# xinntao/EDVR

Measured on AMD Instinct MI355X. Metric: EDVR-L x4 5-frame 720p clips/sec, higher is better.
Workload: dtype fp32 emulated as 2xf16 (hi+lo, 22-bit operands, 4 cross products), fp32 accumulate; 1 GPU; EDVR-L x4, 5 frames, 180x320 LR -> 720x1280, batch 10/GPU, inference; clips_per_gpu=10, global_clips=10, parallelism=clip-sharded x1, no data-path collective, world_size=1, backend=single process

## Files before the change

edvr_amd/_lib.py:

```python
import ctypes
import os

_HERE = os.path.dirname(os.path.abspath(__file__))
LIB_PATH = os.environ.get('EDVR_AMD_LIB') or os.path.join(_HERE, 'lib', 'libedvr_amd.so')

c_float_p = ctypes.c_void_p
i32, i64, f32, sz = ctypes.c_int, ctypes.c_int64, ctypes.c_float, ctypes.c_size_t
vp = ctypes.c_void_p


class ConvDesc(ctypes.Structure):
    _fields_ = [
        ('x1', vp), ('x2', vp), ('c1', i32), ('c2', i32), ('x1_img_stride', i64), ('x2_img_stride', i64),
        ('x2_div', i32), ('x2_mul', i32), ('x2_add', i32), ('n', i32), ('h', i32), ('w', i32), ('wpk', vp),
        ('bias', vp), ('co', i32), ('ks', i32), ('stride', i32), ('act', i32), ('act_from', i32), ('res1', vp),
        ('res2', vp), ('res1_img_stride', i64), ('res2_img_stride', i64), ('y', vp), ('y_img_stride', i64),
        ('out_mode', i32), ('algo', i32), ('gate', vp), ('gate_img_stride', i64), ('gate_slope', f32), ('y_scale', f32),
        ('wpk_f4', vp), ('abs_sum', vp), ('abs_sum_channels', i32), ('wpk_f4s', vp), ('x_amax', vp), ('y_amax', vp),
        ('pre', vp), ('pre_img_stride', i64), ('pre_div', i32), ('pre_mul', i32), ('pre_add', i32), ('pre_n', i32), ('wpk_ds', vp),
    ]


PROTOTYPES = {
    'edvr_version': (ctypes.c_char_p, []),
    'edvr_last_error': (ctypes.c_char_p, []),
    'edvr_check_device': (i32, []),
    'edvr_conv2d_packed_weight_elems': (sz, [i32, i32, i32]),
    'edvr_conv2d_pack_weight_f32': (i32, [vp, vp, i32, i32, i32, i32, vp]),
    'edvr_conv2d_packed_weight_f4_elems': (sz, [i32, i32]),
    'edvr_conv2d_pack_weight_f4_f32': (i32, [vp, vp, i32, i32, i32, vp]),
    'edvr_conv2d_packed_weight_f4s_elems': (sz, [i32, i32]),
    'edvr_conv2d_pack_weight_f4s_f32': (i32, [vp, vp, i32, i32, i32, vp]),
    'edvr_conv2d_packed_weight_1x1s_elems': (sz, [i32, i32]),
    'edvr_conv2d_pack_weight_1x1s_f32': (i32, [vp, vp, i32, i32, vp]),
    'edvr_conv2d_packed_weight_ds_elems': (sz, [i32, i32, i32]),
    'edvr_conv2d_pack_weight_ds_f32': (i32, [vp, vp, i32, i32, i32, vp]),
    'edvr_amax_f32': (i32, [vp, vp, i32, i64, i64, vp]),
    'edvr_pack_job_bytes': (sz, []),
    'edvr_conv2d_pack_weights_multi': (i32, [vp, i32, i32, i32, vp]),
    'edvr_conv2d_f32': (i32, [ctypes.POINTER(ConvDesc), vp]),
    'edvr_conv2d_kernel': (i32, [ctypes.POINTER(ConvDesc)]),
    'edvr_conv2d_gate_supported': (i32, [ctypes.POINTER(ConvDesc)]),
    'edvr_conv2d_abs_sum_supported': (i32, [ctypes.POINTER(ConvDesc)]),
    'edvr_conv2d_y_amax_supported': (i32, [ctypes.POINTER(ConvDesc)]),
    'edvr_conv2d_pre_supported': (i32, [ctypes.POINTER(ConvDesc)]),
    'edvr_conv2d_f4s_set_lean': (i32, [i32]),
    'edvr_conv2d_f4s_lean_items': (i32, [ctypes.POINTER(ConvDesc)]),
    'edvr_conv2d_kernel_name': (i32, [ctypes.POINTER(ConvDesc), ctypes.c_char_p, sz]),
    'edvr_conv2d_executed_flops': (i32, [ctypes.POINTER(ConvDesc), ctypes.POINTER(ctypes.c_double)]),
    'edvr_dcnv2_fwd_ws_bytes': (sz, [i32] * 12),
    'edvr_dcnv2_fwd_f32': (i32, [vp] * 6 + [i32] * 12 + [i64, i64, i32, i32, vp, sz, vp]),
    'edvr_dcnv2_fwd_split_f32': (i32, [vp] * 6 + [i32] * 12 + [i64, i64, i32, i32, vp, sz, vp, vp]),
    'edvr_dcnv2_fwd_split_applies': (i32, [vp] + [i32] * 13),
    'edvr_dcnv2_fwd_kernel_name': (i32, [vp] + [i32] * 13 + [ctypes.c_char_p, sz]),
    'edvr_dcnv2_bwd_ws_bytes': (sz, [i32] * 12),
    'edvr_dcnv2_any_ws_bytes': (sz, [i32] * 13),
    'edvr_dcnv2_fwd_any': (i32, [i32] + [vp] * 6 + [i32] * 12 + [i64, i64, vp, sz, vp]),
    'edvr_dcnv2_bwd_any': (i32, [i32] + [vp] * 10 + [i32] * 12 + [i64, i64, i64, i64, vp, sz, vp]),
    'edvr_psnr_sse_f32': (i32, [vp, vp, vp, i32, i32, i32, i32, i64, i64, i32, i32, i32, vp]),
    'edvr_ssim_partials': (sz, [i32, i32, i32]),
    'edvr_ssim_f32': (i32, [vp, vp, vp, i32, i32, i32, i32, i64, i64, i32, i32, vp]),
    'edvr_niqe_blocks': (sz, [i32, i32, i32]),
    'edvr_niqe_moments_f32': (i32, [vp, vp, i32, i32, i32, i32, i64, i32, vp]),
    'edvr_niqe_moments_u8': (i32, [vp, vp, i32, i32, i32, i64, i32, vp]),
    'edvr_frames_u8_to_f32': (i32, [vp, vp, i32, i32, i32, i32, vp, i32, vp]),
    'edvr_gather_images_f32': (i32, [vp, vp, vp, vp, i32, vp, i32, i32, vp]),
    'edvr_upsample4x_add_u8': (i32, [vp, vp, vp, i32, i32, i32, vp]),
# ... 108 lines not shown
```

edvr_amd/csrc/conv1x1_s.hip:

```cpp
#include <cstdlib>

#include "common.h"
#include "pack.h"

namespace edvr {

typedef float f32x16 __attribute__((ext_vector_type(16)));
typedef int c1s_i32x4 __attribute__((ext_vector_type(4)));
typedef _Float16 c1s_f16x8 __attribute__((ext_vector_type(8)));

struct Conv1x1SArgs {
  edvr_conv2d_desc d;
  const unsigned *wq;
  int ci, cop, co_start;
  int seg_shift;
};

template <int MT>
__global__ __launch_bounds__(256, 2) void conv1x1_split_kernel(const Conv1x1SArgs a) {
  constexpr int CK = 64, MB = 32 * MT, DEPTH = 8, NW = CK * MB / 4 / 256;
  constexpr int RSRC_FLAGS = 0x00020000;
  constexpr int OOB = (int)0x80000000;
  __shared__ __attribute__((aligned(16))) unsigned wsm[2][CK * MB];
  const edvr_conv2d_desc &d = a.d;
  const float s_x = split_scale(__builtin_bit_cast(float, __builtin_amdgcn_readfirstlane(__builtin_bit_cast(int, *d.x_amax))));
  const float inv_sw = __builtin_bit_cast(float, __builtin_amdgcn_readfirstlane((int)a.wq[1]));
  const int tid = threadIdx.x, lane = tid & 63, half = lane >> 5, j = lane & 31;
  const int wave = __builtin_amdgcn_readfirstlane(tid >> 6);
  const int hw = d.h * d.w;
  const int img = blockIdx.z, co_blk = a.co_start + blockIdx.y * MB;
  const int p = (blockIdx.x * 4 + wave) * 32 + j;
  const bool p_ok = p < hw;

  auto uniform_ptr = [&](const float *ptr) {
    const uint64_t pv = reinterpret_cast<uint64_t>(ptr);
    return ((uint64_t)(uint32_t)__builtin_amdgcn_readfirstlane((int)(pv >> 32)) << 32) | (uint32_t)__builtin_amdgcn_readfirstlane((int)(uint32_t)pv);
  };
  const uint64_t b1 = uniform_ptr(d.x1 + (int64_t)img * d.x1_img_stride);
  uint64_t b2 = b1;
  if (d.x2) {
    const int i2 = d.x2_div > 0 ? (img / d.x2_div) * d.x2_mul + d.x2_add : img;
    b2 = uniform_ptr(d.x2 + (int64_t)i2 * d.x2_img_stride);
  }
  const int voff = p_ok ? (4 * half * hw + p) * 4 : OOB;
  const int real_steps = (d.c1 + d.c2) / 8;
  const int seg_mask = (1 << a.seg_shift) - 1;
  const int64_t plane_bytes = (int64_t)hw * 4;
  auto load_b = [&](int s, float (&v)[4]) {
    const int c = 8 * s;
    const bool first = c < d.c1;
    const int cc = first ? c : c - d.c1;
    const uint64_t base = (first ? b1 : b2) + (uint64_t)((int64_t)(cc & ~seg_mask) * plane_bytes);
    const __amdgpu_buffer_rsrc_t rs = __builtin_amdgcn_make_buffer_rsrc(reinterpret_cast<void *>(base), (short)0, 0x7fffffff, RSRC_FLAGS);
    const bool ok = s < real_steps;
#pragma unroll
    for (int i = 0; i < 4; ++i)
      v[i] = __builtin_bit_cast(float, __builtin_amdgcn_raw_buffer_load_b32(rs, ok ? voff : OOB, ok ? ((cc & seg_mask) + i) * hw * 4 : 0, 0));
  };

  const int quads_total = (d.c1 + d.c2 + 3) / 4;
  c1s_i32x4 wr[NW];
  auto w_load = [&](int c0) {
#pragma unroll
    for (int i = 0; i < NW; ++i) {
      const int e = tid + i * 256, q = e / MB, col = e - q * MB;
      const bool ok = c0 / 4 + q < quads_total;
      const c1s_i32x4 v = *reinterpret_cast<const c1s_i32x4 *>(a.wq + 16 + ((int64_t)(ok ? c0 / 4 + q : 0) * a.cop + co_blk + col) * 4);
      wr[i] = ok ? v : c1s_i32x4{0, 0, 0, 0};
    }
  };
  auto w_commit = [&](int buf) {
#pragma unroll
    for (int i = 0; i < NW; ++i) *reinterpret_cast<c1s_i32x4 *>(&wsm[buf][(tid + i * 256) * 4]) = wr[i];
  };

  f32x16 acc[MT];
#pragma unroll
  for (int m = 0; m < MT; ++m)
#pragma unroll
    for (int r = 0; r < 16; ++r) acc[m][r] = 0.f;
  float bq[DEPTH][4];
#pragma unroll
  for (int k = 0; k < DEPTH; ++k) load_b(k, bq[k]);
  w_load(0);
  w_commit(0);
  __syncthreads();

  const int chunks = a.ci / CK;
  for (int ch = 0; ch < chunks; ++ch) {
    const int buf = ch & 1;
    const bool more = ch + 1 < chunks;
    if (more) w_load((ch + 1) * CK);
    const unsigned *ws = wsm[buf] + (half * MB + j) * 4;
#pragma unroll
    for (int s = 0; s < CK / 8; ++s) {
      c1s_i32x4 av[MT];
#pragma unroll
      for (int m = 0; m < MT; ++m) av[m] = *reinterpret_cast<const c1s_i32x4 *>(ws + ((2 * s) * MB + m * 32) * 4);
      unsigned pk[4];
      split4_f16x2(bq[s % DEPTH], s_x, pk);
      load_b(ch * (CK / 8) + s + DEPTH, bq[s % DEPTH]);
      c1s_i32x4 b, br;
#pragma unroll
      for (int q = 0; q < 4; ++q) {
        b[q] = (int)pk[q];
        br[q] = (int)__builtin_amdgcn_alignbit(pk[q], pk[q], 16);
      }
#pragma unroll
      for (int m = 0; m < MT; ++m) acc[m] = __builtin_amdgcn_mfma_f32_32x32x16_f16(__builtin_bit_cast(c1s_f16x8, av[m]), __builtin_bit_cast(c1s_f16x8, b), acc[m], 0, 0, 0);
#pragma unroll
      for (int m = 0; m < MT; ++m) acc[m] = __builtin_amdgcn_mfma_f32_32x32x16_f16(__builtin_bit_cast(c1s_f16x8, av[m]), __builtin_bit_cast(c1s_f16x8, br), acc[m], 0, 0, 0);
      if (s == CK / 16 && more) w_commit(buf ^ 1);
    }
    asm volatile("s_waitcnt lgkmcnt(0)\n\ts_barrier" ::: "memory");
  }

  const float unscale = inv_sw / s_x;
  const float slope = d.act == EDVR_ACT_LRELU ? 0.1f : (d.act == EDVR_ACT_RELU ? 0.f : 1.f);
  const bool sig = d.act == EDVR_ACT_SIGMOID;
  float *y = d.y + (int64_t)img * d.y_img_stride;
  const float *q1 = d.res1 ? d.res1 + (int64_t)img * d.res1_img_stride : nullptr;
  const float *q2 = d.res2 ? d.res2 + (int64_t)img * d.res2_img_stride : nullptr;
  unsigned vmax = 0u;
  if (p_ok) {
#pragma unroll
    for (int m = 0; m < MT; ++m)
#pragma unroll
      for (int r = 0; r < 16; ++r) {
        const int co = co_blk + m * 32 + (r & 3) + 8 * (r >> 2) + 4 * half;
        if (co < d.co) {
          float v = __builtin_fmaf(acc[m][r], unscale, d.bias ? d.bias[co] : 0.f);
          if (co >= d.act_from) v = sig ? __builtin_amdgcn_rcpf(1.f + __expf(-v)) : fmaxf(v, slope * v);
          const int64_t off = (int64_t)co * hw + p;
          if (q1) v += q1[off];
          if (q2) v += q2[off];
          y[off] = v;
          vmax = max(vmax, __builtin_bit_cast(unsigned, v) & 0x7fffffffu);
        }
      }
  }
  if (d.y_amax) {
#pragma unroll
    for (int sh = 32; sh > 0; sh >>= 1) vmax = max(vmax, (unsigned)__shfl_xor((int)vmax, sh));
    if (lane == 0) publish_amax(d.y_amax, vmax);
  }
}

static bool conv1x1_split_enabled() {
  static const bool on = []() {
    const char *e = getenv("EDVR_CONV1X1_SPLIT");
    return !(e && e[0] == '0');
  }();
  return on;
}

bool conv1x1_split_eligible(const edvr_conv2d_desc &d) {
  if (!conv1x1_split_enabled() || !d.wpk_f4s || !d.x_amax || d.algo == EDVR_CONV_DIRECT) return false;
  if (!conv1x1_eligible(d)) return false;
  if ((d.c1 & 7) || (d.c2 & 7)) return false;
  return (int64_t)d.h * d.w * 32 < ((int64_t)1 << 31);
}

int conv1x1_split_launch(const edvr_conv2d_desc &d, hipStream_t stream) {
  EDVR_REQUIRE((reinterpret_cast<uintptr_t>(d.wpk_f4s) & 15) == 0, "conv1x1_split: packed weights must be 16-byte aligned");
  Conv1x1SArgs a;
  a.d = d;
  a.wq = reinterpret_cast<const unsigned *>(d.wpk_f4s);
  a.ci = ((d.c1 + d.c2 + 63) / 64) * 64;
  a.cop = (d.co + 127) / 128 * 128;
  const int hw = d.h * d.w;
  a.seg_shift = 30;
  while (((int64_t)1 << a.seg_shift) * hw * 4 >= ((int64_t)1 << 31)) --a.seg_shift;
  if (a.seg_shift < 3) a.seg_shift = 3;
  const int full = d.co / 128, rem_tiles = cdiv(d.co - full * 128, 32);
  if (full > 0) {
    a.co_start = 0;
    hipLaunchKernelGGL((conv1x1_split_kernel<4>), dim3(cdiv(hw, 128), full, d.n), dim3(256), 0, stream, a);
  }
  if (rem_tiles > 0) {
    a.co_start = full * 128;
    const dim3 grid(cdiv(hw, 128), 1, d.n);
    if (rem_tiles == 1) hipLaunchKernelGGL((conv1x1_split_kernel<1>), grid, dim3(256), 0, stream, a);
    else if (rem_tiles == 2) hipLaunchKernelGGL((conv1x1_split_kernel<2>), grid, dim3(256), 0, stream, a);
    else hipLaunchKernelGGL((conv1x1_split_kernel<3>), grid, dim3(256), 0, stream, a);
  }
  return check_launch("conv1x1_split_kernel");
}

}

extern "C" {

size_t edvr_conv2d_packed_weight_1x1s_elems(int co, int ci) {
  if (co <= 0 || ci <= 0) return 0;
  return 16 + (size_t)((ci + 63) / 64 * 16) * ((co + 127) / 128 * 128) * 4;
}

int edvr_conv2d_pack_weight_1x1s_f32(const float *w, void *wpk, int co, int ci, edvr_stream_t stream_) {
  using namespace edvr;
  EDVR_REQUIRE(w && wpk && co > 0 && ci > 0, "pack_weight_1x1s: bad arguments");
  EDVR_REQUIRE((reinterpret_cast<uintptr_t>(wpk) & 15) == 0, "pack_weight_1x1s: wpk must be 16-byte aligned");
  hipStream_t stream = as_stream(stream_);
  unsigned *wq = static_cast<unsigned *>(wpk);
  const int cop = (co + 127) / 128 * 128, quads = (ci + 63) / 64 * 16;
  return conv_split_pack(w, wq, co, ci, 1, cop, quads, stream);
}

}
```

edvr_amd/edvr_arch.py:

```python
import torch
from torch import nn

from . import functional as F_
from .arch_util import DCNv2Pack, ResidualBlockNoBN, make_layer, warn_offset_absmean

LRELU = F_.ACT_LRELU


def _conv3(cin, cout, stride=1):
    return nn.Conv2d(cin, cout, 3, stride, 1)


class PCDAlignment(nn.Module):

    def __init__(self, num_feat=64, deformable_groups=8):
        super().__init__()
        self.offset_conv1, self.offset_conv2, self.offset_conv3 = nn.ModuleDict(), nn.ModuleDict(), nn.ModuleDict()
        self.dcn_pack, self.feat_conv = nn.ModuleDict(), nn.ModuleDict()
        for lv in (3, 2, 1):
            key = f'l{lv}'
            self.offset_conv1[key] = _conv3(2 * num_feat, num_feat)
            if lv == 3:
                self.offset_conv2[key] = _conv3(num_feat, num_feat)
            else:
# ... 43 lines not shown
        self.temporal_attn1 = _conv3(num_feat, num_feat)
        self.temporal_attn2 = _conv3(num_feat, num_feat)
        self.feat_fusion = nn.Conv2d(num_frame * num_feat, num_feat, 1, 1)
        self.max_pool = nn.MaxPool2d(3, stride=2, padding=1)
        self.avg_pool = nn.AvgPool2d(3, stride=2, padding=1)
        self.spatial_attn1 = nn.Conv2d(num_frame * num_feat, num_feat, 1)
        self.spatial_attn2 = nn.Conv2d(num_feat * 2, num_feat, 1)
        self.spatial_attn3 = _conv3(num_feat, num_feat)
        self.spatial_attn4 = nn.Conv2d(num_feat, num_feat, 1)
        self.spatial_attn5 = _conv3(num_feat, num_feat)
        self.spatial_attn_l1 = nn.Conv2d(num_feat, num_feat, 1)
        self.spatial_attn_l2 = _conv3(num_feat * 2, num_feat)
        self.spatial_attn_l3 = _conv3(num_feat, num_feat)
        self.spatial_attn_add1 = nn.Conv2d(num_feat, num_feat, 1)
        self.spatial_attn_add2 = nn.Conv2d(num_feat, num_feat, 1)
        self.lrelu = nn.LeakyReLU(negative_slope=0.1, inplace=True)
        self.upsample = nn.Upsample(scale_factor=2, mode='bilinear', align_corners=False)

    def forward(self, aligned_feat):
        return self.spatial(self.temporal(aligned_feat))

    def temporal(self, aligned_feat, pair=False):
        b, t, c, h, w = aligned_feat.shape
        alias = F_.ops.carry_bound
        emb_ref = F_.conv(self.temporal_attn1, alias(aligned_feat[:, self.center_frame_idx], aligned_feat))
        emb = F_.conv(self.temporal_attn2, alias(aligned_feat.reshape(b * t, c, h, w), aligned_feat)).view(b, t, -1, h, w)
        if pair:
            mod, mod_rev = F_.tsa_temporal_pair(emb, emb_ref, aligned_feat)
            return alias(mod.view(b, t * c, h, w), mod), alias(mod_rev.view(b, t * c, h, w), mod_rev)
        mod = F_.tsa_temporal(emb, emb_ref, aligned_feat)
        return alias(mod.view(b, t * c, h, w), mod)

    def spatial(self, mod):
        feat = F_.conv(self.feat_fusion, mod, act=LRELU)
        attn = F_.conv(self.spatial_attn1, mod, act=LRELU)
        attn = F_.conv(self.spatial_attn2, F_.pool_maxavg(attn), act=LRELU)
        lvl = F_.conv(self.spatial_attn_l1, attn, act=LRELU)
        lvl = F_.conv(self.spatial_attn_l2, F_.pool_maxavg(lvl), act=LRELU)
        lvl = F_.upsample2x(F_.conv(self.spatial_attn_l3, lvl, act=LRELU))
        attn = F_.conv(self.spatial_attn3, attn, act=LRELU, res1=lvl)
        attn = F_.upsample2x(F_.conv(self.spatial_attn4, attn, act=LRELU))
        attn = F_.conv(self.spatial_attn5, attn)
        attn_add = F_.conv(self.spatial_attn_add2, F_.conv(self.spatial_attn_add1, attn, act=LRELU))
        return F_.tsa_combine(feat, attn, attn_add)


class PredeblurModule(nn.Module):

    def __init__(self, num_in_ch=3, num_feat=64, hr_in=False):
        super().__init__()
        self.hr_in = hr_in
        self.conv_first = _conv3(num_in_ch, num_feat)
        if hr_in:
            self.stride_conv_hr1 = _conv3(num_feat, num_feat, 2)
            self.stride_conv_hr2 = _conv3(num_feat, num_feat, 2)
        self.stride_conv_l2 = _conv3(num_feat, num_feat, 2)
        self.stride_conv_l3 = _conv3(num_feat, num_feat, 2)
        self.resblock_l3 = ResidualBlockNoBN(num_feat=num_feat)
        self.resblock_l2_1 = ResidualBlockNoBN(num_feat=num_feat)
        self.resblock_l2_2 = ResidualBlockNoBN(num_feat=num_feat)
        self.resblock_l1 = nn.ModuleList([ResidualBlockNoBN(num_feat=num_feat) for _ in range(5)])
        self.upsample = nn.Upsample(scale_factor=2, mode='bilinear', align_corners=False)
        self.lrelu = nn.LeakyReLU(negative_slope=0.1, inplace=True)

    def forward(self, x):
        f1 = F_.conv(self.conv_first, x, act=LRELU)
        if self.hr_in:
            f1 = F_.conv(self.stride_conv_hr2, F_.conv(self.stride_conv_hr1, f1, act=LRELU), act=LRELU)
# ... 250 lines not shown
```

edvr_amd/functional.py:

```python
import math
import os

import torch

from . import ops
from .ops import ACT_LRELU, ACT_NONE, ACT_RELU, ACT_SIGMOID, OUT_NCHW, OUT_PIXEL_SHUFFLE2


def _conv_geometry(m):
    ks, st = m.kernel_size, m.stride
    if (ks[0] != ks[1] or ks[0] not in (1, 3) or st[0] != st[1] or st[0] not in (1, 2) or (ks[0] == 1 and st[0] != 1)
            or tuple(m.padding) != (ks[0] // 2, ks[0] // 2) or tuple(m.dilation) != (1, 1) or m.groups != 1):
        raise NotImplementedError(
            f'edvr_amd conv kernel supports 3x3 (stride 1/2, pad 1) and 1x1 convolutions, dilation 1, groups 1; got {m}')
    return ks[0], st[0]


def _needs_grad(*ts):
    return torch.is_grad_enabled() and any(t is not None and t.requires_grad for t in ts)


def conv(m, x, *, x2=None, x2_map=None, act=ACT_NONE, act_from=0, res1=None, res2=None, out_mode=OUT_NCHW, y_scale=1.0,
         abs_sum_channels=0, ci_range=None, use_bias=True, pre=None, pre_map=None, out=None):
    ks, stride = _conv_geometry(m)
# ... 1 lines not shown
        raise ValueError(f'expected a 4-D input, got {tuple(x.shape)}')
    cin = x.shape[1] + (x2.shape[1] if x2 is not None else 0)
    want = m.in_channels if ci_range is None else ci_range[1] - ci_range[0]
    if cin != want:
        raise RuntimeError(f'expected {want} input channels, got {cin}')
    ops.require_gpu(x, x2, m.weight)
    if _needs_grad(x, x2, m.weight, m.bias, res1, res2, pre):
        from . import autograd as ag
        assert abs_sum_channels == 0
        if ci_range is not None or not use_bias or pre is not None or out is not None:
            raise NotImplementedError('ci_range / use_bias / pre / out are inference-only arguments of conv()')
        return ag.conv(m, x, x2, x2_map, act, act_from, res1, res2, out_mode, ks, stride, y_scale)
    wpk = ops.pack_conv_weight(m.weight, ci_range=ci_range)
    f4 = ops.F4_INFERENCE and ks == 3 and stride == 1 and cin >= 32 and m.out_channels >= 48
    f4s = f4 and ops.F4S_INFERENCE and x.shape[3] % 4 == 0
    wf4 = ops.pack_conv_weight(m.weight, f4=True, ci_range=ci_range) if (f4 and not f4s) else None
    wf4s = ops.pack_conv_weight(m.weight, f4s=True, ci_range=ci_range) if f4s else None
    if ops.F4S_INFERENCE and ks == 1 and stride == 1 and cin >= 320 and x.shape[1] % 8 == 0 and cin % 8 == 0:
        wf4s = ops.pack_conv_weight(m.weight, f4s=True, ci_range=ci_range)
    wds = None
    if ops.F4S_INFERENCE and m.out_channels > 4 and (x2 is None or x.shape[1] % 4 == 0) and (
            (ks == 3 and (stride == 2 or cin <= 8)) or (ks == 1 and cin < 320)):
        wds = ops.pack_conv_weight(m.weight, ds=True, ci_range=ci_range)
    bias = m.bias.detach() if (m.bias is not None and use_bias) else None
    r = ops.conv2d(x, wpk, bias, m.out_channels, ks, x2=x2, x2_map=x2_map, stride=stride, act=act, act_from=act_from,
                   res1=res1, res2=res2, out_mode=out_mode, y_scale=y_scale, wpk_f4=wf4, abs_sum_channels=abs_sum_channels,
                   wpk_f4s=wf4s, pre=pre, pre_map=pre_map, out=out, wpk_ds=wds)
    y = r[0] if abs_sum_channels > 0 else r
    if ops.F4S_INFERENCE and ops.get_bound(y) is None:
        ops.linear_bound(y, m.weight, m.bias, (x, x2), (res1, res2, pre), scale=y_scale, floor=1.0 if act == ACT_SIGMOID else 0.0)
    return r


PRE_SPLIT = os.environ.get('EDVR_CONV_PRE', '1') != '0'
PRE_SPLIT_MIN_ITEMS = None


def _conv_items(n, h, w, co):
    return n * -(-co // 64) * min(-(-w // 64) * -(-h // 8), -(-w // 32) * -(-h // 16))


def conv_shared_x2(m, x, x2, x2_map, act=ACT_NONE):
    if PRE_SPLIT and x2_map is not None and x2_map[0] > 1 and not _needs_grad(x, x2, m.weight, m.bias):
        ks, stride = _conv_geometry(m)
        (n, c1, h, w), c2, co = x.shape, x2.shape[1], m.out_channels
        f4 = ops.F4_INFERENCE and ks == 3 and stride == 1 and min(c1, c2) >= 32 and co >= 48
        min_items = PRE_SPLIT_MIN_ITEMS if PRE_SPLIT_MIN_ITEMS is not None else torch.cuda.get_device_properties(x.device).multi_processor_count
        if f4 and _conv_items(n, h, w, co) > min_items and ops.conv_pre_supported(n, c1, h, w, co, ops.F4S_INFERENCE and w % 4 == 0):
            div, mul, add = x2_map
            shared = (n - 1) // div + 1
            sel = x2[add:add + 1] if (mul == 0 or shared == 1) else x2[add:add + (shared - 1) * mul + 1:mul]
            p = conv(m, ops.carry_bound(sel, x2), ci_range=(c1, c1 + c2), use_bias=False)
            return conv(m, x, act=act, ci_range=(0, c1), pre=p, pre_map=(div, 0 if sel.shape[0] == 1 else 1, 0))
    return conv(m, x, x2=x2, x2_map=x2_map, act=act)


def offset_mask_conv_stats(conv_offset, feat):
    co = conv_offset.out_channels
    if _needs_grad(feat, conv_offset.weight, conv_offset.bias):
        om = offset_mask_conv(conv_offset, feat)
        return om, ops.abs_stats_per_image(om.detach()[:, :2 * co // 3])
    return conv(conv_offset, feat, act=ACT_SIGMOID, act_from=2 * co // 3, abs_sum_channels=2 * co // 3)


def offset_mask_conv(conv_offset, feat):
    co = conv_offset.out_channels
# ... 113 lines not shown
```

edvr_amd/ops.py:

```python
import ctypes
import os
import weakref

import torch

from . import _lib
from ._lib import (ACT_LRELU, ACT_NONE, ACT_RELU, ACT_SIGMOID, CONV_AUTO, CONV_DIRECT, CONV_WINOGRAD, CONV_WINOGRAD_F4, CONV_WINOGRAD_F4S, OUT_NCHW,
                   OUT_PIXEL_SHUFFLE2)


def _stream():
    return ctypes.c_void_p(torch.cuda.current_stream().cuda_stream)


def _ptr(t):
    return ctypes.c_void_p(t.data_ptr()) if t is not None else ctypes.c_void_p(0)


def require_gpu(*tensors, dtypes=(torch.float32,)):
    seen = None
    for t in tensors:
        if t is None:
            continue
        if not t.is_cuda:
# ... 542 lines not shown
        else:
            d.wpk_f4s, d.wpk_ds, d.x_amax = None, None, None
    sums = None
    if abs_sum_channels > 0 and L.edvr_conv2d_abs_sum_supported(ctypes.byref(d)):
        sums = torch.zeros(2, n, dtype=torch.float32, device=x1.device)
        d.abs_sum, d.abs_sum_channels = _ptr(sums), int(abs_sum_channels)
    name, flops, nbytes, executed = 'conv2d', 0.0, 0.0, None
    if LAUNCH_HOOK is not None:
        buf = ctypes.create_string_buffer(96)
        L.edvr_conv2d_kernel_name(ctypes.byref(d), buf, 96)
        name = buf.value.decode()
        ex = ctypes.c_double(0.0)
        if L.edvr_conv2d_executed_flops(ctypes.byref(d), ctypes.byref(ex)) == 0:
            executed = ex.value
        flops = 2.0 * n * ho * wo * co * (c1 + d.c2) * ks * ks
        nbytes = 4.0 * (n * (c1 + d.c2) * h * w + n * co * ho * wo * (1 + (res1 is not None) + (res2 is not None) + (gate is not None) + (pre is not None))
                        + co * (c1 + d.c2) * ks * ks)
    _run(name, lambda: _lib.check(L.edvr_conv2d_f32(ctypes.byref(d), _stream()), 'edvr_conv2d_f32'), flops, nbytes, executed)
    if y_bound is not None:
        set_bound(out, y_bound)
    else:
        void_bound(out)
    if abs_sum_channels > 0:
        if sums is None:
            return out, abs_stats_per_image(out[:, :abs_sum_channels])
        step = max(1, n // 4)
        sel = out[::step, :abs_sum_channels]
        r = abs_stats_per_image(sel)
        sums[1, ::step] = r[1] * (float(n) / sel.shape[0])
        return out, sums
    return out


def conv_pre_supported(n, c, h, w, co, f4s, algo=None):
    d = _lib.ConvDesc()
    d.c1, d.n, d.h, d.w, d.co, d.ks, d.stride = c, n, h, w, co, 3, 1
    d.algo = CONV_ALGO if algo is None else algo
    any_ptr = ctypes.addressof(d) & ~15
    if f4s:
        d.wpk_f4s = d.x_amax = any_ptr
    else:
        d.wpk_f4 = any_ptr
    return bool(_lib.lib().edvr_conv2d_pre_supported(ctypes.byref(d)))


def conv_gate_supported(n, c, h, w, co, algo=None):
    d = _lib.ConvDesc()
    d.c1, d.n, d.h, d.w, d.co, d.ks, d.stride = c, n, h, w, co, 3, 1
    d.algo = CONV_ALGO if algo is None else algo
    return bool(_lib.lib().edvr_conv2d_gate_supported(ctypes.byref(d)))


def _ones_mask(offset):
    return torch.ones(offset.shape[0], offset.shape[1] // 2, offset.shape[2], offset.shape[3], dtype=offset.dtype, device=offset.device)


def dcnv1_forward(x, offset, weight, stride, pad, dil, groups, dg, halo_hint=0, out=None):
    if require_gpu(x, offset, weight, dtypes=tuple(DCN_DTYPES)) != torch.float32:
        return dcnv2_forward(x, offset, _ones_mask(offset), weight, None, stride, pad, dil, groups, dg, out=out)
    L = _lib.lib()
    offset = _as_planes(offset)
    dims = _dcn_dims(x, weight, stride, pad, dil, groups, dg)
    B, C, H, W, Co, kh, kw = dims[:7]
    ho, wo = offset.shape[2], offset.shape[3]
    if out is not None:
        if tuple(out.shape) != (B, Co, ho, wo) or out.dtype != torch.float32 or not out.is_contiguous() or out.device != x.device:
# ... 1228 lines not shown
```

include/edvr_amd.h:

```cpp
#ifndef EDVR_AMD_H
#define EDVR_AMD_H

#include <stddef.h>
#include <stdint.h>

#ifdef __cplusplus
extern "C" {
#endif

#define EDVR_OK 0
#define EDVR_ERR_ARG (-1)
#define EDVR_ERR_UNSUPPORTED (-2)
#define EDVR_ERR_LAUNCH (-3)
#define EDVR_ERR_WORKSPACE (-4)

typedef void *edvr_stream_t;

const char *edvr_version(void);
const char *edvr_last_error(void);
int edvr_check_device(void);

#define EDVR_ACT_NONE 0
#define EDVR_ACT_RELU 1
#define EDVR_ACT_LRELU 2
// ... 30 lines not shown
  const float *res1;
  const float *res2;
  int64_t res1_img_stride, res2_img_stride;
  float *y;
  int64_t y_img_stride;
  int out_mode;
  int algo;
  const float *gate;
  int64_t gate_img_stride;
  float gate_slope;
  float y_scale;
  const float *wpk_f4;
  float *abs_sum;
  int abs_sum_channels;
  const void *wpk_f4s;
  const float *x_amax;
  float *y_amax;
  const float *pre;
  int64_t pre_img_stride;
  int pre_div, pre_mul, pre_add;
  int pre_n;
  const void *wpk_ds;
} edvr_conv2d_desc;

size_t edvr_conv2d_packed_weight_elems(int co, int ci, int ks);
int edvr_conv2d_pack_weight_f32(const float *w, float *wpk, int co, int ci, int ks, int transpose_flip,
                                edvr_stream_t stream);
size_t edvr_conv2d_packed_weight_f4_elems(int co, int ci);
int edvr_conv2d_pack_weight_f4_f32(const float *w, float *wpk_f4, int co, int ci, int transpose_flip, edvr_stream_t stream);
size_t edvr_conv2d_packed_weight_f4s_elems(int co, int ci);
int edvr_conv2d_pack_weight_f4s_f32(const float *w, void *wpk_f4s, int co, int ci, int transpose_flip, edvr_stream_t stream);
size_t edvr_conv2d_packed_weight_1x1s_elems(int co, int ci);
int edvr_conv2d_pack_weight_1x1s_f32(const float *w, void *wpk_1x1s, int co, int ci, edvr_stream_t stream);
size_t edvr_conv2d_packed_weight_ds_elems(int co, int ci, int ks);
int edvr_conv2d_pack_weight_ds_f32(const float *w, void *wpk_ds, int co, int ci, int ks, edvr_stream_t stream);
int edvr_amax_f32(const float *x, float *amax, int n, int64_t per_img, int64_t img_stride, edvr_stream_t stream);
size_t edvr_pack_job_bytes(void);
int edvr_conv2d_pack_weights_multi(const void *jobs, int n_jobs, int total_blocks, int split_parity, edvr_stream_t stream);
int edvr_conv2d_f32(const edvr_conv2d_desc *d, edvr_stream_t stream);
#define EDVR_CONV_KERNEL_SMALL 0
#define EDVR_CONV_KERNEL_F4S 1
#define EDVR_CONV_KERNEL_F4 2
#define EDVR_CONV_KERNEL_F2 3
#define EDVR_CONV_KERNEL_1X1_SPLIT 4
#define EDVR_CONV_KERNEL_1X1_STREAM 5
#define EDVR_CONV_KERNEL_DIRECT_SPLIT 6
#define EDVR_CONV_KERNEL_DIRECT 7
int edvr_conv2d_kernel(const edvr_conv2d_desc *d);
int edvr_conv2d_gate_supported(const edvr_conv2d_desc *d);
int edvr_conv2d_y_amax_supported(const edvr_conv2d_desc *d);
int edvr_conv2d_abs_sum_supported(const edvr_conv2d_desc *d);
int edvr_conv2d_pre_supported(const edvr_conv2d_desc *d);
int edvr_conv2d_f4s_set_lean(int on);
int edvr_conv2d_f4s_lean_items(const edvr_conv2d_desc *d);
int edvr_conv2d_kernel_name(const edvr_conv2d_desc *d, char *buf, size_t buf_len);
int edvr_conv2d_executed_flops(const edvr_conv2d_desc *d, double *flops);

#define EDVR_HW(h, w) ((int)(h) | (((int)(w) + 1) << 16))

size_t edvr_dcnv2_fwd_ws_bytes(int B, int C, int H, int W, int Co, int kh, int kw, int stride, int pad, int dil,
                               int groups, int dg);
int edvr_dcnv2_fwd_f32(const float *x, const float *offset, const float *mask, const float *weight,
                       const float *bias, float *y, int B, int C, int H, int W, int Co, int kh, int kw, int stride,
                       int pad, int dil, int groups, int dg, int64_t offset_bstride, int64_t mask_bstride, int act,
                       int halo_hint, void *ws, size_t ws_bytes, edvr_stream_t stream);

// ... 214 lines not shown
```

Measured before the change: 106.8 clips/s.

## Fuse TSA feat_fusion and spatial_attn1 1x1 convs into one two-head kernel

Adds a two-head variant of the split-f16 1x1 conv kernel that reads the shared input once and computes both the feat_fusion and spatial_attn1 outputs in one launch, each with its own weights, bias, activation and amax slot. The TSA fusion module now calls conv_pair instead of two separate convs. The goal is to halve input reads and drop a launch for these two large 1x1 convs over the concatenated frame features. In exchange, the workgroup now holds up to eight 32-channel tiles, so chunk size drops to 32 and register pressure rises, which may reduce occupancy.

Result: no change. 107.2 clips/s (median of 6 runs) (+0.4%).

```diff
diff --git a/edvr_amd/_lib.py b/edvr_amd/_lib.py
--- a/edvr_amd/_lib.py
+++ b/edvr_amd/_lib.py
@@ -33,6 +33,8 @@
     'edvr_conv2d_pack_weight_f4s_f32': (i32, [vp, vp, i32, i32, i32, vp]),
     'edvr_conv2d_packed_weight_1x1s_elems': (sz, [i32, i32]),
     'edvr_conv2d_pack_weight_1x1s_f32': (i32, [vp, vp, i32, i32, vp]),
+    'edvr_conv1x1_split_heads_supported': (i32, [ctypes.POINTER(ConvDesc), ctypes.POINTER(ConvDesc)]),
+    'edvr_conv1x1_split_heads_f32': (i32, [ctypes.POINTER(ConvDesc), ctypes.POINTER(ConvDesc), vp]),
     'edvr_conv2d_packed_weight_ds_elems': (sz, [i32, i32, i32]),
     'edvr_conv2d_pack_weight_ds_f32': (i32, [vp, vp, i32, i32, i32, vp]),
     'edvr_amax_f32': (i32, [vp, vp, i32, i64, i64, vp]),
diff --git a/edvr_amd/csrc/conv1x1_s.hip b/edvr_amd/csrc/conv1x1_s.hip
--- a/edvr_amd/csrc/conv1x1_s.hip
+++ b/edvr_amd/csrc/conv1x1_s.hip
@@ -14,11 +14,18 @@
   const unsigned *wq;
   int ci, cop, co_start;
   int seg_shift;
+  const unsigned *wq2;
+  const float *bias2;
+  float *y2, *y2_amax;
+  int64_t y2_img_stride;
+  int co2, cop2, act2, act_from2, mt1;
 };
 
-template <int MT>
+template <int MT, int HEADS>
 __global__ __launch_bounds__(256, 2) void conv1x1_split_kernel(const Conv1x1SArgs a) {
-  constexpr int CK = 64, MB = 32 * MT, DEPTH = 8, NW = CK * MB / 4 / 256;
+  constexpr int CK = MT > 4 ? 32 : 64, MB = 32 * MT, DEPTH = 8, NW = CK * MB / 4 / 256;
+  constexpr int SPC = CK / 8, CPI = DEPTH / SPC;
+  static_assert(HEADS == 2 || MT <= 4, "one head: up to four tiles per workgroup, further blocks on grid.y");
   constexpr int RSRC_FLAGS = 0x00020000;
   constexpr int OOB = (int)0x80000000;
   __shared__ __attribute__((aligned(16))) unsigned wsm[2][CK * MB];
@@ -65,7 +72,13 @@
     for (int i = 0; i < NW; ++i) {
       const int e = tid + i * 256, q = e / MB, col = e - q * MB;
       const bool ok = c0 / 4 + q < quads_total;
-      const c1s_i32x4 v = *reinterpret_cast<const c1s_i32x4 *>(a.wq + 16 + ((int64_t)(ok ? c0 / 4 + q : 0) * a.cop + co_blk + col) * 4);
+      c1s_i32x4 v;
+      if constexpr (HEADS == 2) {
+        const bool h2 = col >= 32 * a.mt1;
+        v = *reinterpret_cast<const c1s_i32x4 *>((h2 ? a.wq2 : a.wq) + 16 + ((int64_t)(ok ? c0 / 4 + q : 0) * (h2 ? a.cop2 : a.cop) + (h2 ? col - 32 * a.mt1 : col)) * 4);
+      } else {
+        v = *reinterpret_cast<const c1s_i32x4 *>(a.wq + 16 + ((int64_t)(ok ? c0 / 4 + q : 0) * a.cop + co_blk + col) * 4);
+      }
       wr[i] = ok ? v : c1s_i32x4{0, 0, 0, 0};
     }
   };
@@ -87,34 +100,93 @@
   __syncthreads();
 
   const int chunks = a.ci / CK;
-  for (int ch = 0; ch < chunks; ++ch) {
-    const int buf = ch & 1;
-    const bool more = ch + 1 < chunks;
-    if (more) w_load((ch + 1) * CK);
-    const unsigned *ws = wsm[buf] + (half * MB + j) * 4;
-#pragma unroll
-    for (int s = 0; s < CK / 8; ++s) {
-      c1s_i32x4 av[MT];
-#pragma unroll
-      for (int m = 0; m < MT; ++m) av[m] = *reinterpret_cast<const c1s_i32x4 *>(ws + ((2 * s) * MB + m * 32) * 4);
-      unsigned pk[4];
-      split4_f16x2(bq[s % DEPTH], s_x, pk);
-      load_b(ch * (CK / 8) + s + DEPTH, bq[s % DEPTH]);
-      c1s_i32x4 b, br;
-#pragma unroll
-      for (int q = 0; q < 4; ++q) {
-        b[q] = (int)pk[q];
-        br[q] = (int)__builtin_amdgcn_alignbit(pk[q], pk[q], 16);
-      }
-#pragma unroll
-      for (int m = 0; m < MT; ++m) acc[m] = __builtin_amdgcn_mfma_f32_32x32x16_f16(__builtin_bit_cast(c1s_f16x8, av[m]), __builtin_bit_cast(c1s_f16x8, b), acc[m], 0, 0, 0);
-#pragma unroll
-      for (int m = 0; m < MT; ++m) acc[m] = __builtin_amdgcn_mfma_f32_32x32x16_f16(__builtin_bit_cast(c1s_f16x8, av[m]), __builtin_bit_cast(c1s_f16x8, br), acc[m], 0, 0, 0);
-      if (s == CK / 16 && more) w_commit(buf ^ 1);
+  for (int it = 0; it < a.ci / (8 * DEPTH); ++it) {
+#pragma unroll
+    for (int c = 0; c < CPI; ++c) {
+      const int ch = it * CPI + c;
+      const int buf = ch & 1;
+      const bool more = ch + 1 < chunks;
+      if (more) w_load((ch + 1) * CK);
+      const unsigned *ws = wsm[buf] + (half * MB + j) * 4;
+#pragma unroll
+      for (int s = 0; s < SPC; ++s) {
+        constexpr int MG = MT > 4 ? 4 : MT;
+        c1s_i32x4 av[MT];
+#pragma unroll
+        for (int m = 0; m < MG; ++m) av[m] = *reinterpret_cast<const c1s_i32x4 *>(ws + ((2 * s) * MB + m * 32) * 4);
+        unsigned pk[4];
+        split4_f16x2(bq[c * SPC + s], s_x, pk);
+        load_b(ch * SPC + s + DEPTH, bq[c * SPC + s]);
+        c1s_i32x4 b, br;
+#pragma unroll
+        for (int q = 0; q < 4; ++q) {
+          b[q] = (int)pk[q];
+          br[q] = (int)__builtin_amdgcn_alignbit(pk[q], pk[q], 16);
+        }
+        constexpr bool LATE = MT == 7;
+        if constexpr (!LATE) {
+#pragma unroll
+          for (int m = MG; m < MT; ++m) av[m] = *reinterpret_cast<const c1s_i32x4 *>(ws + ((2 * s) * MB + m * 32) * 4);
+        }
+#pragma unroll
+        for (int m0 = 0; m0 < MT; m0 += MG) {
+          if constexpr (LATE) {
+            if (m0 > 0) {
+#pragma unroll
+              for (int m = MG; m < MT; ++m) av[m] = *reinterpret_cast<const c1s_i32x4 *>(ws + ((2 * s) * MB + m * 32) * 4);
+            }
+          }
+#pragma unroll
+          for (int m = m0; m < m0 + MG && m < MT; ++m) acc[m] = __builtin_amdgcn_mfma_f32_32x32x16_f16(__builtin_bit_cast(c1s_f16x8, av[m]), __builtin_bit_cast(c1s_f16x8, b), acc[m], 0, 0, 0);
+#pragma unroll
+          for (int m = m0; m < m0 + MG && m < MT; ++m) acc[m] = __builtin_amdgcn_mfma_f32_32x32x16_f16(__builtin_bit_cast(c1s_f16x8, av[m]), __builtin_bit_cast(c1s_f16x8, br), acc[m], 0, 0, 0);
+        }
+        if (s == SPC / 2 && more) w_commit(buf ^ 1);
+      }
+      asm volatile("s_waitcnt lgkmcnt(0)\n\ts_barrier" ::: "memory");
     }
-    asm volatile("s_waitcnt lgkmcnt(0)\n\ts_barrier" ::: "memory");
-  }
-
+  }
+
+  if constexpr (HEADS == 2) {
+    const float inv_sw2 = __builtin_bit_cast(float, __builtin_amdgcn_readfirstlane((int)a.wq2[1]));
+    unsigned vmax[2] = {0u, 0u};
+    if (p_ok) {
+#pragma unroll
+      for (int m = 0; m < MT; ++m) {
+        const bool h2 = m >= a.mt1;
+        const float unscale = (h2 ? inv_sw2 : inv_sw) / s_x;
+        const int act = h2 ? a.act2 : d.act, act_from = h2 ? a.act_from2 : d.act_from, co_n = h2 ? a.co2 : d.co;
+        const float slope = act == EDVR_ACT_LRELU ? 0.1f : (act == EDVR_ACT_RELU ? 0.f : 1.f);
+        const bool sig = act == EDVR_ACT_SIGMOID;
+        const float *bias = h2 ? a.bias2 : d.bias;
+        float *y = h2 ? a.y2 + (int64_t)img * a.y2_img_stride : d.y + (int64_t)img * d.y_img_stride;
+        unsigned vm = 0u;
+#pragma unroll
+        for (int r = 0; r < 16; ++r) {
+          const int co = (h2 ? m - a.mt1 : m) * 32 + (r & 3) + 8 * (r >> 2) + 4 * half;
+          if (co < co_n) {
+            float v = __builtin_fmaf(acc[m][r], unscale, bias ? bias[co] : 0.f);
+            if (co >= act_from) v = sig ? __builtin_amdgcn_rcpf(1.f + __expf(-v)) : fmaxf(v, slope * v);
+            y[(int64_t)co * hw + p] = v;
+            vm = max(vm, __builtin_bit_cast(unsigned, v) & 0x7fffffffu);
+          }
+        }
+        vmax[0] = max(vmax[0], h2 ? 0u : vm);
+        vmax[1] = max(vmax[1], h2 ? vm : 0u);
+      }
+    }
+#pragma unroll
+    for (int hd = 0; hd < 2; ++hd) {
+      float *slot = hd ? a.y2_amax : d.y_amax;
+      if (slot) {
+        unsigned v = vmax[hd];
+#pragma unroll
+        for (int sh = 32; sh > 0; sh >>= 1) v = max(v, (unsigned)__shfl_xor((int)v, sh));
+        if (lane == 0) publish_amax(slot, v);
+      }
+    }
+    return;
+  }
   const float unscale = inv_sw / s_x;
   const float slope = d.act == EDVR_ACT_LRELU ? 0.1f : (d.act == EDVR_ACT_RELU ? 0.f : 1.f);
   const bool sig = d.act == EDVR_ACT_SIGMOID;
@@ -161,9 +233,8 @@
   return (int64_t)d.h * d.w * 32 < ((int64_t)1 << 31);
 }
 
-int conv1x1_split_launch(const edvr_conv2d_desc &d, hipStream_t stream) {
-  EDVR_REQUIRE((reinterpret_cast<uintptr_t>(d.wpk_f4s) & 15) == 0, "conv1x1_split: packed weights must be 16-byte aligned");
-  Conv1x1SArgs a;
+static Conv1x1SArgs conv1x1_split_args(const edvr_conv2d_desc &d) {
+  Conv1x1SArgs a = {};
   a.d = d;
   a.wq = reinterpret_cast<const unsigned *>(d.wpk_f4s);
   a.ci = ((d.c1 + d.c2 + 63) / 64) * 64;
@@ -172,19 +243,72 @@
   a.seg_shift = 30;
   while (((int64_t)1 << a.seg_shift) * hw * 4 >= ((int64_t)1 << 31)) --a.seg_shift;
   if (a.seg_shift < 3) a.seg_shift = 3;
+  return a;
+}
+
+int conv1x1_split_launch(const edvr_conv2d_desc &d, hipStream_t stream) {
+  EDVR_REQUIRE((reinterpret_cast<uintptr_t>(d.wpk_f4s) & 15) == 0, "conv1x1_split: packed weights must be 16-byte aligned");
+  Conv1x1SArgs a = conv1x1_split_args(d);
+  const int hw = d.h * d.w;
   const int full = d.co / 128, rem_tiles = cdiv(d.co - full * 128, 32);
   if (full > 0) {
     a.co_start = 0;
-    hipLaunchKernelGGL((conv1x1_split_kernel<4>), dim3(cdiv(hw, 128), full, d.n), dim3(256), 0, stream, a);
+    hipLaunchKernelGGL((conv1x1_split_kernel<4, 1>), dim3(cdiv(hw, 128), full, d.n), dim3(256), 0, stream, a);
   }
   if (rem_tiles > 0) {
     a.co_start = full * 128;
     const dim3 grid(cdiv(hw, 128), 1, d.n);
-    if (rem_tiles == 1) hipLaunchKernelGGL((conv1x1_split_kernel<1>), grid, dim3(256), 0, stream, a);
-    else if (rem_tiles == 2) hipLaunchKernelGGL((conv1x1_split_kernel<2>), grid, dim3(256), 0, stream, a);
-    else hipLaunchKernelGGL((conv1x1_split_kernel<3>), grid, dim3(256), 0, stream, a);
+    if (rem_tiles == 1) hipLaunchKernelGGL((conv1x1_split_kernel<1, 1>), grid, dim3(256), 0, stream, a);
+    else if (rem_tiles == 2) hipLaunchKernelGGL((conv1x1_split_kernel<2, 1>), grid, dim3(256), 0, stream, a);
+    else hipLaunchKernelGGL((conv1x1_split_kernel<3, 1>), grid, dim3(256), 0, stream, a);
   }
   return check_launch("conv1x1_split_kernel");
+}
+
+static bool conv1x1_split_takes(const edvr_conv2d_desc &d) {
+  if (!conv1x1_split_enabled() || !d.x1 || !d.y || !d.wpk_f4s || !d.x_amax || (reinterpret_cast<uintptr_t>(d.wpk_f4s) & 15)) return false;
+  if (d.ks != 1 || d.stride != 1 || d.out_mode != EDVR_OUT_NCHW || d.gate || d.pre || d.abs_sum) return false;
+  if (d.y_scale != 0.f && d.y_scale != 1.f) return false;
+  if (d.n <= 0 || d.n > 65535 || d.h <= 0 || d.w <= 0 || d.co <= 0 || d.c1 <= 0 || (d.x2 != nullptr) != (d.c2 > 0)) return false;
+  if ((d.c1 & 7) || (d.c2 & 7)) return false;
+  return (int64_t)d.h * d.w * 32 < ((int64_t)1 << 31);
+}
+
+static bool conv1x1_split_same_input(const edvr_conv2d_desc &a, const edvr_conv2d_desc &b) {
+  return a.x1 == b.x1 && a.x2 == b.x2 && a.c1 == b.c1 && a.c2 == b.c2 && a.x1_img_stride == b.x1_img_stride && a.x2_img_stride == b.x2_img_stride &&
+         a.x2_div == b.x2_div && a.x2_mul == b.x2_mul && a.x2_add == b.x2_add && a.n == b.n && a.h == b.h && a.w == b.w && a.x_amax == b.x_amax;
+}
+
+static bool conv1x1_split_heads_fit(const edvr_conv2d_desc &a, const edvr_conv2d_desc &b) {
+  if (!conv1x1_split_takes(a) || !conv1x1_split_takes(b) || !conv1x1_split_same_input(a, b)) return false;
+  if (a.res1 || a.res2 || b.res1 || b.res2) return false;
+  return cdiv(a.co, 32) + cdiv(b.co, 32) <= 8;
+}
+
+static int conv1x1_split_heads_launch(const edvr_conv2d_desc &da, const edvr_conv2d_desc &db, hipStream_t stream) {
+  Conv1x1SArgs a = conv1x1_split_args(da);
+  a.co_start = 0;
+  a.wq2 = reinterpret_cast<const unsigned *>(db.wpk_f4s);
+  a.bias2 = db.bias;
+  a.y2 = db.y;
+  a.y2_amax = db.y_amax;
+  a.y2_img_stride = db.y_img_stride;
+  a.co2 = db.co;
+  a.cop2 = (db.co + 127) / 128 * 128;
+  a.act2 = db.act;
+  a.act_from2 = db.act_from;
+  a.mt1 = cdiv(da.co, 32);
+  const dim3 grid(cdiv(da.h * da.w, 128), 1, da.n);
+  switch (a.mt1 + cdiv(db.co, 32)) {
+    case 2: hipLaunchKernelGGL((conv1x1_split_kernel<2, 2>), grid, dim3(256), 0, stream, a); break;
+    case 3: hipLaunchKernelGGL((conv1x1_split_kernel<3, 2>), grid, dim3(256), 0, stream, a); break;
+    case 4: hipLaunchKernelGGL((conv1x1_split_kernel<4, 2>), grid, dim3(256), 0, stream, a); break;
+    case 5: hipLaunchKernelGGL((conv1x1_split_kernel<5, 2>), grid, dim3(256), 0, stream, a); break;
+    case 6: hipLaunchKernelGGL((conv1x1_split_kernel<6, 2>), grid, dim3(256), 0, stream, a); break;
+    case 7: hipLaunchKernelGGL((conv1x1_split_kernel<7, 2>), grid, dim3(256), 0, stream, a); break;
+    default: hipLaunchKernelGGL((conv1x1_split_kernel<8, 2>), grid, dim3(256), 0, stream, a); break;
+  }
+  return check_launch("conv1x1_split_kernel (two heads)");
 }
 
 }
@@ -206,4 +330,19 @@
   return conv_split_pack(w, wq, co, ci, 1, cop, quads, stream);
 }
 
-}
+int edvr_conv1x1_split_heads_supported(const edvr_conv2d_desc *a, const edvr_conv2d_desc *b) {
+  if (!a) return 0;
+  return (b ? edvr::conv1x1_split_heads_fit(*a, *b) : edvr::conv1x1_split_takes(*a)) ? 1 : 0;
+}
+
+int edvr_conv1x1_split_heads_f32(const edvr_conv2d_desc *a, const edvr_conv2d_desc *b, edvr_stream_t stream) {
+  using namespace edvr;
+  EDVR_REQUIRE(a != nullptr, "conv1x1_split_heads: null descriptor");
+  if (!edvr_conv1x1_split_heads_supported(a, b)) {
+    set_error("conv1x1_split_heads: not a launch of the split 1x1 kernel (ask edvr_conv1x1_split_heads_supported)");
+    return EDVR_ERR_UNSUPPORTED;
+  }
+  return b ? conv1x1_split_heads_launch(*a, *b, as_stream(stream)) : conv1x1_split_launch(*a, as_stream(stream));
+}
+
+}
diff --git a/edvr_amd/edvr_arch.py b/edvr_amd/edvr_arch.py
--- a/edvr_amd/edvr_arch.py
+++ b/edvr_amd/edvr_arch.py
@@ -99,8 +99,7 @@
         return alias(mod.view(b, t * c, h, w), mod)
 
     def spatial(self, mod):
-        feat = F_.conv(self.feat_fusion, mod, act=LRELU)
-        attn = F_.conv(self.spatial_attn1, mod, act=LRELU)
+        feat, attn = F_.conv_pair(self.feat_fusion, self.spatial_attn1, mod, LRELU, LRELU)
         attn = F_.conv(self.spatial_attn2, F_.pool_maxavg(attn), act=LRELU)
         lvl = F_.conv(self.spatial_attn_l1, attn, act=LRELU)
         lvl = F_.conv(self.spatial_attn_l2, F_.pool_maxavg(lvl), act=LRELU)
diff --git a/edvr_amd/functional.py b/edvr_amd/functional.py
--- a/edvr_amd/functional.py
+++ b/edvr_amd/functional.py
@@ -57,6 +57,21 @@
     return r
 
 
+TWO_HEADS = os.environ.get('EDVR_CONV1X1_TWO_HEADS', '1') != '0'
+
+
+def conv_pair(m_a, m_b, x, act_a=ACT_NONE, act_b=ACT_NONE):
+    if (TWO_HEADS and ops.F4S_INFERENCE and x.dim() == 4 and not _needs_grad(x, m_a.weight, m_a.bias, m_b.weight, m_b.bias)
+            and all(_conv_geometry(m) == (1, 1) and m.in_channels == x.shape[1] for m in (m_a, m_b))):
+        ops.require_gpu(x, m_a.weight, m_b.weight)
+        heads = [(ops.pack_conv_weight(m.weight, f4s=True), m.bias.detach() if m.bias is not None else None, m.out_channels, act, 0)
+                 for m, act in ((m_a, act_a), (m_b, act_b))]
+        r = ops.conv1x1_split_heads(x, heads)
+        if r is not None:
+            return r[0], r[1]
+    return conv(m_a, x, act=act_a), conv(m_b, x, act=act_b)
+
+
 PRE_SPLIT = os.environ.get('EDVR_CONV_PRE', '1') != '0'
 PRE_SPLIT_MIN_ITEMS = None
 
diff --git a/edvr_amd/ops.py b/edvr_amd/ops.py
--- a/edvr_amd/ops.py
+++ b/edvr_amd/ops.py
@@ -598,6 +598,60 @@
     return out
 
 
+def conv1x1_split_heads(x1, heads, *, x2=None, x2_map=None, x_amax=None, algo=None, direct=False):
+    assert len(heads) in (1, 2)
+    require_gpu(x1, x2, *[h[1] for h in heads])
+    require_gpu(*[h[0] for h in heads], dtypes=(torch.int32,))
+    L = _lib.lib()
+    x1_in, x2_in = x1, x2
+    x1 = _as_planes(x1)
+    n, c1, h, w = x1.shape
+    if x2 is not None:
+        x2 = _as_planes(x2)
+    descs, outs = [], []
+    for wq, bias, co, act, act_from in heads:
+        d = _lib.ConvDesc()
+        d.x1, d.c1, d.x1_img_stride = _ptr(x1), c1, _img_stride(x1)
+        if x2 is not None:
+            d.x2, d.c2, d.x2_img_stride = _ptr(x2), x2.shape[1], _img_stride(x2)
+            if x2_map is not None:
+                d.x2_div, d.x2_mul, d.x2_add = x2_map
+        d.n, d.h, d.w, d.co, d.ks, d.stride = n, h, w, co, 1, 1
+        d.bias, d.act, d.act_from, d.out_mode, d.y_scale = _ptr(bias), act, act_from, OUT_NCHW, 1.0
+        d.algo = CONV_ALGO if algo is None else algo
+        d.wpk_f4s = _ptr(wq)
+        d.x_amax = d.y = _ptr(heads[0][0])
+        descs.append(d)
+    second = ctypes.byref(descs[1]) if len(descs) > 1 else None
+    if not L.edvr_conv1x1_split_heads_supported(ctypes.byref(descs[0]), second):
+        return None
+    if not direct and any(L.edvr_conv2d_kernel(ctypes.byref(d)) != _lib.CONV_KERNEL_1X1_SPLIT for d in descs):
+        return None
+    if x_amax is None:
+        x_amax = input_bound(x1_in, x1)
+        if x2 is not None:
+            x_amax = torch.maximum(x_amax, input_bound(x2_in, x2))
+    require_gpu(x_amax)
+    if BOUND_CHECK:
+        true = amax(x1).item() if x2 is None else max(amax(x1).item(), amax(x2).item())
+        if not (x_amax.item() >= true):
+            raise AssertionError(f'magnitude bound {x_amax.item():.6g} < max |x| = {true:.6g} for a conv input of shape {tuple(x1.shape)}')
+        BOUND_CHECK_LOG.extend([(tuple(x1.shape), x_amax.item() / max(true, 1e-30))] * len(descs))
+    bounds = []
+    for d in descs:
+        out = torch.empty((n, d.co, h, w), dtype=torch.float32, device=x1.device)
+        bounds.append(_arena(x1.device).slot(x1.device))
+        d.x_amax, d.y, d.y_img_stride, d.y_amax = _ptr(x_amax), _ptr(out), _img_stride(out), _ptr(bounds[-1])
+        outs.append(out)
+    ci, co_all = c1 + descs[0].c2, sum(d.co for d in descs)
+    name = 'conv1x1_split_kernel' if len(descs) == 1 else 'conv1x1_split_kernel[two heads]'
+    _run(name, lambda: _lib.check(L.edvr_conv1x1_split_heads_f32(ctypes.byref(descs[0]), second, _stream()), 'edvr_conv1x1_split_heads_f32'),
+         2.0 * n * h * w * co_all * ci, 4.0 * (n * ci * h * w + n * co_all * h * w + co_all * ci), 8.0 * n * h * w * co_all * ci)
+    for out, b in zip(outs, bounds):
+        set_bound(out, b)
+    return outs
+
+
 def conv_pre_supported(n, c, h, w, co, f4s, algo=None):
     d = _lib.ConvDesc()
     d.c1, d.n, d.h, d.w, d.co, d.ks, d.stride = c, n, h, w, co, 3, 1
diff --git a/include/edvr_amd.h b/include/edvr_amd.h
--- a/include/edvr_amd.h
+++ b/include/edvr_amd.h
@@ -86,6 +86,8 @@
 int edvr_conv2d_pack_weight_f4s_f32(const float *w, void *wpk_f4s, int co, int ci, int transpose_flip, edvr_stream_t stream);
 size_t edvr_conv2d_packed_weight_1x1s_elems(int co, int ci);
 int edvr_conv2d_pack_weight_1x1s_f32(const float *w, void *wpk_1x1s, int co, int ci, edvr_stream_t stream);
+int edvr_conv1x1_split_heads_supported(const edvr_conv2d_desc *a, const edvr_conv2d_desc *b);
+int edvr_conv1x1_split_heads_f32(const edvr_conv2d_desc *a, const edvr_conv2d_desc *b, edvr_stream_t stream);
 size_t edvr_conv2d_packed_weight_ds_elems(int co, int ci, int ks);
 int edvr_conv2d_pack_weight_ds_f32(const float *w, void *wpk_ds, int co, int ci, int ks, edvr_stream_t stream);
 int edvr_amax_f32(const float *x, float *amax, int n, int64_t per_img, int64_t img_stride, edvr_stream_t stream);
```
